# intellect4all/storage-engines

Measured on AMD Instinct MI355X. Metric: bloom build+probe Mkeys/s device-resident, 10M×16B keys @1% FPR, 1/2/4/8 GPU, higher is better.
Workload: dtype u64

## Files before the change

storage-engines_amd/csrc/seb_bucket.hip:

```cpp
#include <hip/hip_runtime.h>
#include <math.h>
#include <stdint.h>

#include "seb_device.h"
#include "seb_kernels.h"

namespace seb {

constexpr int kBktShift = 16;
constexpr uint32_t kBktWords = 1u << (kBktShift - 5);
constexpr uint32_t kMaxBuckets = 4096;
constexpr uint32_t kTilePos = 28672;
constexpr uint32_t kMaxTiles = 1024;
constexpr uint32_t kTargetTiles = 256;

__device__ __forceinline__ uint32_t block_exclusive_scan(uint32_t x, uint32_t *wsum, uint32_t *total) {
    const uint32_t lane = threadIdx.x & 63, wid = threadIdx.x >> 6, nw = blockDim.x >> 6;
    uint32_t v = x;
#pragma unroll
    for (int d = 1; d < 64; d <<= 1) {
        uint32_t y = __shfl_up(v, d, 64);
        if (lane >= (uint32_t)d) v += y;
    }
    if (lane == 63) wsum[wid] = v;
// ... 56 lines not shown
    for (uint64_t k0 = t0; k0 < t1; k0 += round_keys) {
        const uint64_t k1 = k0 + round_keys < t1 ? k0 + round_keys : t1;
        uint32_t pos[KP][KQ];
        bool valid[KP];
        if constexpr (KFIX > 0) {
#pragma unroll
            for (int r = 0; r < KP; ++r) {
                const uint64_t i = k0 + (uint64_t)r * blockDim.x + threadIdx.x;
                valid[r] = i < k1;
                if (valid[r]) {
                    if constexpr (IsPacked<Src>::value) {
                        static_assert(KFIX == 7, "packed residues are k == 7");
                        packed_positions((uint64_t)kv[r].x | (uint64_t)kv[r].y << 32, (uint32_t)md.m, (uint32_t)md.c,
                                         pos[r]);
                    } else {
                        uint64_t h1, h2;
                        if constexpr (kPre)
                            Src::hash_raw(kv[r], h1, h2);
                        else
                            src.hash(i, h1, h2);
                        for_positions<KFIX, true>(h1, h2, md, KFIX,
                                                  [&](uint32_t q, uint64_t p) { pos[r][q] = (uint32_t)p; });
                    }
#pragma unroll
                    for (int q = 0; q < KQ; ++q) atomicAdd(&cursor[pos[r][q] >> kBktShift], 1u);
                }
            }
            if (k1 < t1) prefetch(k1);
        } else {
            for (uint64_t i = k0 + threadIdx.x; i < k1; i += blockDim.x) {
                uint64_t h1, h2;
                src.hash(i, h1, h2);
                for_positions<0, true>(h1, h2, md, md.k,
                                       [&](uint32_t, uint64_t p) { atomicAdd(&cursor[(uint32_t)p >> kBktShift], 1u); });
            }
        }
        __syncthreads();
        {
            const uint32_t b0 = threadIdx.x * per;
            uint32_t c[8] = {0u, 0u, 0u, 0u, 0u, 0u, 0u, 0u}, s = 0;
            for (uint32_t j = 0; j < per; ++j)
                if (b0 + j < nb) {
                    c[j] = cursor[b0 + j];
                    s += c[j];
                }
            uint32_t tot;
            uint32_t pre = block_exclusive_scan(s, wsum, &tot);
            for (uint32_t j = 0; j < per; ++j)
                if (b0 + j < nb) {
                    cursor[b0 + j] = pre;
                    pre += c[j];
                }
        }
        __syncthreads();
        if constexpr (KFIX > 0) {
            uint32_t slot[KP][KQ];
#pragma unroll
            for (int r = 0; r < KP; ++r)
                if (valid[r]) {
#pragma unroll
                    for (int q = 0; q < KQ; ++q) slot[r][q] = atomicAdd(&cursor[pos[r][q] >> kBktShift], 1u);
                }
#pragma unroll
            for (int r = 0; r < KP; ++r)
                if (valid[r]) {
#pragma unroll
                    for (int q = 0; q < KQ; ++q) sorted[slot[r][q]] = pos[r][q];
                }
        } else {
            for (uint64_t i = k0 + threadIdx.x; i < k1; i += blockDim.x) {
                uint64_t h1, h2;
                src.hash(i, h1, h2);
                for_positions<0, true>(h1, h2, md, md.k, [&](uint32_t, uint64_t p) {
                    sorted[atomicAdd(&cursor[(uint32_t)p >> kBktShift], 1u)] = (uint32_t)p;
                });
            }
        }
        __syncthreads();
        for (uint32_t b = threadIdx.x; b < nb; b += blockDim.x) {
            const uint32_t start = b ? cursor[b - 1] : 0u, c = cursor[b] - start;
            const uint32_t reg = b * ntiles + t;
            if (fill[b] + c > cap) *ovf = 1u;
            fill[b] = reg * cap + fill[b] - start;
        }
        __syncthreads();
        const uint32_t cnt = (uint32_t)(k1 - k0) * md.k;
        if (*ovf == 0u) {
#pragma unroll 5
            for (uint32_t idx = threadIdx.x; idx < cnt; idx += blockDim.x) {
                const uint32_t p = sorted[idx];
                regions[fill[p >> kBktShift] + idx] = (uint16_t)p;
            }
        } else {
            for (uint32_t idx = threadIdx.x; idx < cnt; idx += blockDim.x) {
                const uint32_t p = sorted[idx];
                const uint32_t b = p >> kBktShift;
                const uint32_t e = fill[b] + idx;
                if (e - (b * ntiles + t) * cap < cap)
                    regions[e] = (uint16_t)p;
                else
                    __hip_atomic_fetch_or(ovw + (p >> 5), 1u << (p & 31), __ATOMIC_RELAXED, __HIP_MEMORY_SCOPE_AGENT);
            }
        }
        __syncthreads();
        for (uint32_t b = threadIdx.x; b < nb; b += blockDim.x) {
            fill[b] += cursor[b] - (b * ntiles + t) * cap;
            cursor[b] = 0u;
        }
        if (threadIdx.x == 0) *ovf = 0u;
        __syncthreads();
    }
    for (uint32_t b = threadIdx.x; b < nb; b += blockDim.x) counts[(uint64_t)b * ntiles + t] = fill[b];
}

constexpr uint32_t kBinMinBuckets = 512;
constexpr uint32_t kBinBig = 48, kBinSmall = 32;
constexpr uint32_t bin_lds_bytes(uint32_t nb, uint32_t slots) { return nb * (slots * 2 + 8) + 16; }
constexpr uint32_t kBinBigMaxBuckets = (160u * 1024 - 16) / (kBinBig * 2 + 8);
constexpr uint32_t kBinMaxBuckets = (160u * 1024 - 16) / (kBinSmall * 2 + 8);
constexpr double kBinMeanPos[2] = {20.0, 25.0};

__device__ __forceinline__ void bins_overflow_or(uint32_t *ovw, uint32_t b, uint32_t l) {
    const uint32_t p = (b << kBktShift) | l;
    __hip_atomic_fetch_or(ovw + (p >> 5), 1u << (p & 31), __ATOMIC_RELAXED, __HIP_MEMORY_SCOPE_AGENT);
}

template <typename Src, int THREADS, int KPT, uint32_t SB, int G = 1>
__global__ __launch_bounds__(THREADS) void k_bkt_scatter_bins(Src src, uint64_t n, ModArg md, uint32_t nb,
                                                              uint32_t tile_keys, uint32_t round_keys, uint32_t ntiles,
                                                              uint32_t cap, uint16_t *__restrict__ regions,
                                                              uint32_t *__restrict__ counts, uint32_t *__restrict__ ovw) {
    extern __shared__ uint4 smem4[];
    constexpr uint32_t S = SB, PAD = 8;
    static_assert(S % 8 == 0 && S <= 64, "a bucket's chunks must sit in one wave");
    uint16_t *bins = (uint16_t *)smem4;
    uint32_t *cnt = (uint32_t *)(bins + (size_t)nb * S);
    uint32_t *fill = cnt + nb;
    const uint32_t t = blockIdx.x;
    for (uint32_t b = threadIdx.x; b < nb; b += THREADS) {
        cnt[b] = 0u;
        fill[b] = 0u;
    }
    __syncthreads();
    const uint64_t t0 = (uint64_t)t * tile_keys;
    const uint64_t t1 = t0 + tile_keys < n ? t0 + tile_keys : n;
    constexpr bool kPre = SplitLoad<Src>::value;
    uint4 kv[kPre ? KPT : 1];
    auto prefetch = [&](uint64_t r0) {
        if constexpr (kPre) {
            const uint64_t r1 = r0 + round_keys < t1 ? r0 + round_keys : t1;
#pragma unroll
            for (int r = 0; r < KPT; ++r) {
                const uint64_t i = r0 + (uint64_t)r * THREADS + threadIdx.x;
                if (i < r1) kv[r] = src.load(i);
            }
        }
    };
    prefetch(t0);
    for (uint64_t k0 = t0; k0 < t1; k0 += round_keys) {
        const uint64_t k1 = k0 + round_keys < t1 ? k0 + round_keys : t1;
        constexpr int NSTEP = (KPT + G - 1) / G;
        uint32_t pp[G][7], ps[G][7];
        bool pv[G];
#pragma unroll
        for (int g = 0; g < G; ++g) pv[g] = false;
        auto write_bins = [&](const uint32_t (&pw)[7], const uint32_t (&sw)[7]) {
#pragma unroll
            for (int q = 0; q < 7; ++q) {
                const uint32_t p = pw[q], sl = sw[q], b = p >> kBktShift;
                bins[sl < S ? b * S + sl : nb * S + 4 * nb] = (uint16_t)p;
                if (sl >= S) {
                    const uint32_t e = fill[b] + sl;
                    if (e < cap)
                        regions[(uint64_t)(b * ntiles + t) * cap + e] = (uint16_t)p;
                    else
                        bins_overflow_or(ovw, b, p & 0xffffu);
                }
            }
        };
#pragma unroll
        for (int st = 0; st < NSTEP; ++st) {
            uint32_t pos[G][7], sl[G][7];
            bool valid[G];
#pragma unroll
            for (int g = 0; g < G; ++g) {
                const int r = st * G + g;
                const uint64_t i = k0 + (uint64_t)r * THREADS + threadIdx.x;
                valid[g] = r < KPT && i < k1;
                if (r < KPT && (kPre || valid[g])) {
                    if constexpr (IsPacked<Src>::value) {
                        packed_positions((uint64_t)kv[r].x | (uint64_t)kv[r].y << 32, (uint32_t)md.m, (uint32_t)md.c,
                                         pos[g]);
                    } else {
                        uint64_t h1, h2;
                        if constexpr (kPre)
                            Src::hash_raw(kv[r], h1, h2);
                        else
                            src.hash(i, h1, h2);
                        for_positions<7, true>(h1, h2, md, 7, [&](uint32_t q, uint64_t p) { pos[g][q] = (uint32_t)p; });
                    }
                }
            }
#pragma unroll
            for (int g = 0; g < G; ++g) {
                const int r = st * G + g;
                if (r >= KPT) continue;
                const uint64_t i = k0 + (uint64_t)r * THREADS + threadIdx.x;
                if constexpr (kPre) {
                    const uint64_t in = i + round_keys;
                    if (valid[g] && k1 < t1 && in < (k1 + round_keys < t1 ? k1 + round_keys : t1)) kv[r] = src.load(in);
                }
                if (valid[g]) {
#pragma unroll
                    for (int q = 0; q < 7; ++q) sl[g][q] = atomicAdd(&cnt[pos[g][q] >> kBktShift], 1u);
                }
            }
#pragma unroll
            for (int g = 0; g < G; ++g) {
                if (pv[g]) write_bins(pp[g], ps[g]);
#pragma unroll
                for (int q = 0; q < 7; ++q) {
                    pp[g][q] = pos[g][q];
                    ps[g][q] = sl[g][q];
                }
                pv[g] = valid[g];
            }
        }
#pragma unroll
        for (int g = 0; g < G; ++g)
            if (pv[g]) write_bins(pp[g], ps[g]);
        __syncthreads();
        {
            constexpr uint32_t NCH = S / 8, BPW = 64 / NCH, NW = THREADS / 64;
            const uint32_t lane = threadIdx.x & 63u, g = lane / NCH, j = lane - g * NCH;
            for (uint32_t b0 = (threadIdx.x >> 6) * BPW; b0 < nb; b0 += NW * BPW) {
                const uint32_t b = b0 + g;
                if (g >= BPW || b >= nb) continue;
                const uint32_t c = cnt[b], f = fill[b];
                const uint32_t rb = (b * ntiles + t) * cap;
                if (j * 8 < c) {
                    const uint4 w = *(const uint4 *)(bins + b * S + j * 8);
                    const uint32_t live = c - j * 8;
                    uint32_t ww[4] = {w.x, w.y, w.z, w.w};
                    const uint32_t e0 = w.x & 0xffffu, hi0 = e0 << 16;
#pragma unroll
                    for (uint32_t i = 0; i < 4; ++i)
                        ww[i] = 2 * i + 1 < live ? ww[i] : 2 * i < live ? (ww[i] & 0xffffu) | hi0 : e0 | hi0;
                    const uint32_t e = f + j * 8;
                    if (e < cap) {
                        *(uint4 *)(regions + rb + e) = make_uint4(ww[0], ww[1], ww[2], ww[3]);
                    } else {
#pragma unroll
                        for (uint32_t i = 0; i < 8; ++i) bins_overflow_or(ovw, b, (ww[i >> 1] >> ((i & 1) * 16)) & 0xffffu);
                    }
                }
                if (j == 0) {
                    const uint32_t padded = (c + (PAD - 1)) & ~(PAD - 1);
                    if (c > S) {
                        const uint16_t d = bins[b * S];
                        for (uint32_t e = f + c; e < f + padded; ++e)
                            if (e < cap) regions[(uint64_t)rb + e] = d;
                    }
                    cnt[b] = 0u;
                    fill[b] = f + padded;
                }
            }
        }
        __syncthreads();
    }
    for (uint32_t b = threadIdx.x; b < nb; b += THREADS) counts[(uint64_t)b * ntiles + t] = fill[b];
}

template <int THREADS, bool FRESH, bool PADDED = false>
__global__ __launch_bounds__(THREADS) void k_bkt_apply(const uint16_t *__restrict__ regions,
                                                   const uint32_t *__restrict__ counts, uint32_t ntiles, uint32_t cap,
                                                   uint32_t *__restrict__ words, uint64_t nwords,
                                                   uint32_t *__restrict__ ovf) {
    __shared__ uint32_t img[kBktWords];
    __shared__ uint32_t cnt[kMaxTiles];
    __shared__ uint32_t spilled, longest;
    const uint32_t b = blockIdx.x;
    for (uint32_t j = threadIdx.x; j < kBktWords; j += blockDim.x) img[j] = 0u;
    if (threadIdx.x == 0) {
        spilled = 0u;
        longest = 0u;
    }
    __syncthreads();
    for (uint32_t t = threadIdx.x; t < ntiles; t += blockDim.x) {
        const uint32_t c = counts[(uint64_t)b * ntiles + t];
        if (c > cap) spilled = 1u;
        cnt[t] = min(c, cap);
        atomicMax(&longest, min(c, cap));
    }
    __syncthreads();
    const uint32_t stride = cap / 8;
    const uint32_t chunks = (longest + 7) / 8;
    const uint32_t pairs = ntiles * chunks;
    const uint4 *reg = (const uint4 *)(regions + (uint64_t)b * ntiles * cap);
    constexpr uint32_t U = 4;
    for (uint32_t q0 = threadIdx.x; q0 < pairs; q0 += U * THREADS) {
        uint4 v[U];
#pragma unroll
        for (uint32_t u = 0; u < U; ++u) {
            const uint32_t q = q0 + u * THREADS;
            if (q < pairs) {
                const uint32_t t = q / chunks, c = q - t * chunks;
                v[u] = reg[t * stride + c];
            }
        }
#pragma unroll
        for (uint32_t u = 0; u < U; ++u) {
            const uint32_t q = q0 + u * THREADS;
            if (q >= pairs) break;
            const uint32_t t = q / chunks, c = q - t * chunks;
            const uint32_t valid = cnt[t];
            if (c * 8 < valid) {
                const uint32_t w[4] = {v[u].x, v[u].y, v[u].z, v[u].w};
#pragma unroll
                for (uint32_t e = 0; e < 8; ++e)
                    if (PADDED || c * 8 + e < valid) {
                        const uint32_t l = (w[e >> 1] >> ((e & 1) * 16)) & 0xffffu;
                        atomicOr(&img[l >> 5], 1u << (l & 31));
                    }
            }
        }
    }
    __syncthreads();
    const uint64_t w0 = (uint64_t)b * kBktWords;
    if constexpr (FRESH) {
        const bool sp = spilled != 0u;
        for (uint32_t j = threadIdx.x; j < kBktWords; j += blockDim.x)
            if (w0 + j < nwords) {
                uint32_t v = img[j];
                if (sp) {
                    v |= ovf[w0 + j];
                    ovf[w0 + j] = 0u;
                }
                words[w0 + j] = v;
            }
    } else {
        for (uint32_t j = threadIdx.x; j < kBktWords; j += blockDim.x) {
            const uint32_t v = img[j];
            if (v && w0 + j < nwords) words[w0 + j] |= v;
        }
    }
}


struct BktPlan {
    uint32_t nb, tile_keys, ntiles, cap;
    uint32_t round_keys;
    uint32_t bins;
    uint64_t off_regions, off_counts, bytes;
};

static uint32_t bin_slots(uint64_t m, uint32_t k) {
    const uint64_t nb = ((m + 31) / 32 + kBktWords - 1) / kBktWords;
    if (k != 7 || nb < kBinMinBuckets || nb > kBinMaxBuckets) return 0;
    return nb <= kBinBigMaxBuckets ? kBinBig : kBinSmall;
}
static uint32_t use_bins(uint64_t m, uint32_t k) { return options().scatter_bins ? bin_slots(m, k) : 0; }

constexpr uint32_t kScatterThreads = 1024;
static uint32_t scatter_kpt(uint32_t nb) {
    return ((uint64_t)kScatterThreads * 5 * 7 + 2 * nb + 17) * 4 <= 160u * 1024 ? 5u : 4u;
}

static BktPlan plan_bucketed(uint64_t n, uint64_t m, uint32_t k, uint32_t bins) {
    BktPlan p{};
    const uint64_t nwords = (m + 31) / 32;
    p.nb = (uint32_t)((nwords + kBktWords - 1) / kBktWords);
    p.bins = bins;
    const uint32_t thr = kScatterThreads;
    const uint32_t kpt = bins ? 5u : scatter_kpt(p.nb);
    const uint32_t pos = thr * kpt * 7;
    uint32_t round_keys = k == 7 ? kpt * thr : pos / k;
    if (bins) {
        const double mean = kBinMeanPos[bins == kBinBig];
        const uint64_t most = (uint64_t)(mean * (double)m / (double)(1u << kBktShift) / k);
        if (most < round_keys) round_keys = (uint32_t)(most > 64 ? most : 64);
    }
    const uint32_t target = kTargetTiles;
    uint64_t rounds_total = (n + round_keys - 1) / round_keys;
// ... 117 lines not shown
```

storage-engines_amd/csrc/seb_device.h:

```cpp
#pragma once
#include <hip/hip_runtime.h>
#include <stdint.h>

#include <type_traits>

#include "seb_kernels.h"

namespace seb {

constexpr uint64_t kFnvOffset = 0xcbf29ce484222325ull;
constexpr uint64_t kFnvPrime = 0x100000001b3ull;


__device__ __forceinline__ void fnv_byte(uint32_t b, uint64_t &h1, uint64_t &h2) {
    h1 = (h1 ^ (uint64_t)b) * kFnvPrime;
    h2 = (h2 * kFnvPrime) ^ (uint64_t)b;
}

__device__ __forceinline__ void fnv_word(uint32_t w, uint64_t &h1, uint64_t &h2) {
    fnv_byte(w & 0xffu, h1, h2);
    fnv_byte((w >> 8) & 0xffu, h1, h2);
    fnv_byte((w >> 16) & 0xffu, h1, h2);
    fnv_byte(w >> 24, h1, h2);
}
// ... 40 lines not shown
            break;
        default:
            asm("v_xor_b32_sdwa %0, %1, %2 dst_sel:DWORD dst_unused:UNUSED_PAD src0_sel:BYTE_3 src1_sel:DWORD"
                : "=v"(r) : "v"(w), "v"(a));
            break;
    }
    return r;
}

__device__ __forceinline__ void fnv_key16(const uint4 v, uint64_t &h1, uint64_t &h2) {
    const uint32_t w[4] = {v.x, v.y, v.z, v.w};
    uint32_t lo1 = (uint32_t)kFnvOffset, lo2 = (uint32_t)kFnvOffset;
    uint64_t acc1 = (uint32_t)(kFnvOffset >> 32) * pow435(16), acc2 = acc1;
#pragma unroll
    for (int j = 0; j < 16; ++j) {
        const uint32_t x = xor_byte(lo1, w[j >> 2], j & 3);
        const uint64_t p = (uint64_t)x * 435u;
        lo1 = (uint32_t)p;
        acc1 = mad_lo((uint32_t)(p >> 32) + (x << 8), pow435(15 - j), acc1);
        const uint64_t q = (uint64_t)lo2 * 435u;
        acc2 = mad_lo((uint32_t)(q >> 32) + (lo2 << 8), pow435(15 - j), acc2);
        lo2 = xor_byte((uint32_t)q, w[j >> 2], j & 3);
    }
    h1 = (acc1 << 32) | lo1;
    h2 = (acc2 << 32) | lo2;
}

struct FnvSplit {
    uint32_t lo1 = (uint32_t)kFnvOffset, lo2 = (uint32_t)kFnvOffset;
    uint64_t a1 = kFnvOffset >> 32, a2 = kFnvOffset >> 32;
    __device__ __forceinline__ void word(uint32_t w) {
        uint32_t d1[4], d2[4];
#pragma unroll
        for (int j = 0; j < 4; ++j) {
            const uint32_t x = xor_byte(lo1, w, j);
            const uint64_t p = (uint64_t)x * 435u;
            lo1 = (uint32_t)p;
            d1[j] = (uint32_t)(p >> 32) + (x << 8);
            const uint64_t q = (uint64_t)lo2 * 435u;
            d2[j] = (uint32_t)(q >> 32) + (lo2 << 8);
            lo2 = xor_byte((uint32_t)q, w, j);
        }
        const uint64_t t1 = mad_lo(d1[0], pow435(3), mad_lo(d1[1], pow435(2), mad_lo(d1[2], 435u, d1[3])));
        const uint64_t t2 = mad_lo(d2[0], pow435(3), mad_lo(d2[1], pow435(2), mad_lo(d2[2], 435u, d2[3])));
        a1 = mad_lo((uint32_t)a1, pow435(4), t1);
        a2 = mad_lo((uint32_t)a2, pow435(4), t2);
    }
    __device__ __forceinline__ void get(uint64_t &h1, uint64_t &h2) const {
        h1 = (a1 << 32) | lo1;
        h2 = (a2 << 32) | lo2;
    }
};

struct Keys16 {
    static constexpr bool kSplit = true;
    const uint4 *p;
    __device__ __forceinline__ uint64_t index(uint64_t i) const { return i; }
    __device__ __forceinline__ uint4 load(uint64_t i) const {
        typedef unsigned int u32x4 __attribute__((ext_vector_type(4)));
        const u32x4 v = __builtin_nontemporal_load((const u32x4 *)(p + i));
        return make_uint4(v.x, v.y, v.z, v.w);
    }
    __device__ __forceinline__ static void hash_raw(const uint4 v, uint64_t &h1, uint64_t &h2) { fnv_key16(v, h1, h2); }
    __device__ __forceinline__ void hash(uint64_t i, uint64_t &h1, uint64_t &h2) const { fnv_key16(load(i), h1, h2); }
};

struct KeysStrideW {
    const uint32_t *p;
    uint32_t words;
    __device__ __forceinline__ uint64_t index(uint64_t i) const { return i; }
    __device__ __forceinline__ void hash(uint64_t i, uint64_t &h1, uint64_t &h2) const {
        const uint32_t *k = p + i * words;
        h1 = kFnvOffset;
        h2 = kFnvOffset;
        for (uint32_t j = 0; j < words; ++j) fnv_word(k[j], h1, h2);
    }
};

struct KeysStrideB {
    const uint8_t *p;
    uint32_t stride;
    __device__ __forceinline__ uint64_t index(uint64_t i) const { return i; }
    __device__ __forceinline__ void hash(uint64_t i, uint64_t &h1, uint64_t &h2) const {
        const uint8_t *k = p + i * stride;
        h1 = kFnvOffset;
        h2 = kFnvOffset;
        for (uint32_t j = 0; j < stride; ++j) fnv_byte(k[j], h1, h2);
    }
};

__device__ __forceinline__ void fnv_range(const uint8_t *p, uint64_t s, uint64_t e, uint64_t &h1, uint64_t &h2) {
    h1 = kFnvOffset;
    h2 = kFnvOffset;
    uintptr_t a = ((uintptr_t)(p + s)) & ~(uintptr_t)3;
    const uintptr_t end = (uintptr_t)(p + e);
    const uintptr_t beg = (uintptr_t)(p + s);
    for (; a < end; a += 4) {
        const uint32_t w = *(const uint32_t *)a;
        const uint32_t lo = beg > a ? (uint32_t)(beg - a) : 0u;
        const uint32_t hi = end - a < 4 ? (uint32_t)(end - a) : 4u;
        if (lo == 0 && hi == 4)
            fnv_word(w, h1, h2);
        else
            fnv_word_part(w, lo, hi, h1, h2);
    }
}

struct KeysVar {
    const uint8_t *p;
    const uint64_t *off;
    __device__ __forceinline__ uint64_t index(uint64_t i) const { return i; }
    __device__ __forceinline__ void hash(uint64_t i, uint64_t &h1, uint64_t &h2) const {
        fnv_range(p, off[i], off[i + 1], h1, h2);
    }
};

struct KeysHashed {
    static constexpr bool kSplit = true;
    const uint4 *h;
    __device__ __forceinline__ uint64_t index(uint64_t i) const { return i; }
    __device__ __forceinline__ uint4 load(uint64_t i) const { return h[i]; }
    __device__ __forceinline__ static void hash_raw(const uint4 v, uint64_t &h1, uint64_t &h2) {
        h1 = (uint64_t)v.x | ((uint64_t)v.y << 32);
        h2 = (uint64_t)v.z | ((uint64_t)v.w << 32);
    }
    __device__ __forceinline__ void hash(uint64_t i, uint64_t &h1, uint64_t &h2) const { hash_raw(h[i], h1, h2); }
};

template <typename S, typename = void>
struct SplitLoad { static constexpr bool value = false; };
template <typename S>
struct SplitLoad<S, std::void_t<decltype(S::kSplit)>> { static constexpr bool value = S::kSplit; };


__device__ __forceinline__ uint64_t mod64(uint64_t x, uint64_t m, uint64_t mu) {
    uint64_t q = __umul64hi(x, mu);
    uint64_t r = x - q * m;
    r = r >= m ? r - m : r;
    r = r >= m ? r - m : r;
    return r;
}

__device__ __forceinline__ uint32_t mod_m31(uint64_t x, uint32_t m, uint64_t mu) {
    const uint32_t xl = (uint32_t)x, xh = (uint32_t)(x >> 32);
    const uint32_t ul = (uint32_t)mu, uh = (uint32_t)(mu >> 32);
    const uint64_t a = (uint64_t)xh * ul + __umulhi(xl, ul);
    const uint64_t b = (uint64_t)xl * uh + (uint32_t)a;
    const uint32_t qlo = xh * uh + (uint32_t)(a >> 32) + (uint32_t)(b >> 32);
    const uint32_t r = xl - qlo * m;
    const uint32_t s = r - m;
    return s < r ? s : r;
}

template <int KFIX, bool M32, typename F>
__device__ __forceinline__ void for_positions(uint64_t h1, uint64_t h2, const ModArg &md, uint32_t krt, F &&f) {
    const uint32_t k = KFIX > 0 ? (uint32_t)KFIX : krt;
    if (k == 0) return;
    uint64_t x = h1;
    if constexpr (M32) {
        const uint32_t m = (uint32_t)md.m, c = (uint32_t)md.c;
        uint32_t r = mod_m31(h1, m, md.mu);
        const uint32_t b = mod_m31(h2, m, md.mu);
        const uint32_t nb = m - b;
        const uint32_t bc = b >= c ? b - c : b + (m - c);
        const uint32_t nd = m - bc;
        f(0u, (uint64_t)r);
#pragma unroll
        for (uint32_t i = 1; i < k; ++i) {
            uint64_t xn = x + h2;
            const bool carry = xn < x;
            x = xn;
            const uint32_t na = carry ? nd : nb;
            const uint32_t t = r - na;
            r = r >= na ? t : t + m;
            f(i, (uint64_t)r);
        }
    } else {
        const uint64_t m = md.m, c = md.c;
        uint64_t r = mod64(h1, md.m, md.mu);
        const uint64_t b = mod64(h2, md.m, md.mu);
        f(0u, r);
#pragma unroll
        for (uint32_t i = 1; i < k; ++i) {
            uint64_t xn = x + h2;
            bool carry = xn < x;
            x = xn;
            uint64_t s = r + b;
            s = (s < r || s >= m) ? s - m : s;
            uint64_t t = s >= c ? s - c : s + (m - c);
            r = carry ? t : s;
            f(i, r);
        }
    }
}

template <typename Fn>
static inline hipError_t with_src(const KeyBatch &kb, Fn &&fn) {
    if (kb.hashes) return fn(KeysHashed{kb.hashes});
    if (kb.offsets) return fn(KeysVar{kb.data, kb.offsets});
    if (kb.stride == 16 && ((uintptr_t)kb.data & 15) == 0) return fn(Keys16{(const uint4 *)kb.data});
    if (kb.stride % 4 == 0 && ((uintptr_t)kb.data & 3) == 0)
        return fn(KeysStrideW{(const uint32_t *)kb.data, kb.stride / 4});
    return fn(KeysStrideB{kb.data, kb.stride});
}

__device__ __forceinline__ uint64_t pack_residue(uint64_t h1, uint64_t h2, const ModArg &md) {
    const uint64_t r0 = mod_m31(h1, (uint32_t)md.m, md.mu), b = mod_m31(h2, (uint32_t)md.m, md.mu);
    uint64_t f = 0, x = h1;
#pragma unroll
    for (uint32_t q = 1; q < 7; ++q) {
        const uint64_t xn = x + h2;
        f |= (uint64_t)(xn < x) << (q - 1);
        x = xn;
    }
    return r0 | (b << kPackBits) | (f << (2 * kPackBits));
}

__device__ __forceinline__ void packed_positions(uint64_t v, uint32_t m, uint32_t c, uint32_t pos[7]) {
    constexpr uint64_t kMask = (1ull << kPackBits) - 1;
    uint32_t x = (uint32_t)(v & kMask);
    const uint32_t b = (uint32_t)((v >> kPackBits) & kMask), f = (uint32_t)(v >> (2 * kPackBits));
    const uint32_t nb = m - b, bc = b >= c ? b - c : b + (m - c), nd = m - bc;
    pos[0] = x;
#pragma unroll
    for (int q = 1; q < 7; ++q) {
        const uint32_t na = (f >> (q - 1)) & 1u ? nd : nb;
        const uint32_t t = x - na;
        x = x >= na ? t : t + m;
        pos[q] = x;
    }
}

__device__ __forceinline__ uint64_t pack_residue6(uint64_t h1, uint64_t h2, const ModArg &md) {
    const uint64_t r0 = mod_m31(h1, (uint32_t)md.m, md.mu), b = mod_m31(h2, (uint32_t)md.m, md.mu);
    uint64_t f = 0, x = h1;
#pragma unroll
    for (uint32_t q = 1; q < 7; ++q) {
        const uint64_t xn = x + h2;
        f |= (uint64_t)(xn < x) << (q - 1);
        x = xn;
    }
    return r0 | (b << kPack6Bits) | (f << (2 * kPack6Bits));
}
__device__ __forceinline__ void store_packed6(uint8_t *base, uint64_t i, uint64_t v) {
    const uint64_t blk = i >> 6;
    const uint32_t lane = (uint32_t)i & 63u;
    __builtin_nontemporal_store((uint32_t)v, (uint32_t *)(base + blk * kPack6Block) + lane);
    __builtin_nontemporal_store((uint16_t)(v >> 32), (uint16_t *)(base + blk * kPack6Block + 256) + lane);
}
__device__ __forceinline__ uint64_t load_packed6(const uint8_t *base, uint64_t i) {
    const uint64_t blk = i >> 6;
    const uint32_t lane = (uint32_t)i & 63u;
    const uint32_t lo = __builtin_nontemporal_load((const uint32_t *)(base + blk * kPack6Block) + lane);
    const uint16_t hi = __builtin_nontemporal_load((const uint16_t *)(base + blk * kPack6Block + 256) + lane);
    return (uint64_t)lo | ((uint64_t)hi << 32);
}

struct KeysPacked {
    static constexpr bool kSplit = true;
    static constexpr bool kPacked = true;
    const uint64_t *p;
    __device__ __forceinline__ uint64_t index(uint64_t i) const { return i; }
    __device__ __forceinline__ uint4 load(uint64_t i) const {
        const uint64_t v = __builtin_nontemporal_load(p + i);
        return make_uint4((uint32_t)v, (uint32_t)(v >> 32), 0u, 0u);
    }
};

template <typename S, typename = void>
struct IsPacked { static constexpr bool value = false; };
template <typename S>
struct IsPacked<S, std::void_t<decltype(S::kPacked)>> { static constexpr bool value = S::kPacked; };

__device__ __forceinline__ uint64_t wave_peers(bool live, uint32_t v, uint32_t bits) {
    uint64_t peers = __ballot(live);
    for (uint32_t b = 0; b < bits; ++b) {
        const uint64_t on = __ballot(live && ((v >> b) & 1u));
        peers &= ((v >> b) & 1u) ? on : ~on;
    }
    return peers;
}

__device__ __forceinline__ uint32_t lanes_below(uint64_t mask) {
    return __builtin_amdgcn_mbcnt_hi((uint32_t)(mask >> 32), __builtin_amdgcn_mbcnt_lo((uint32_t)mask, 0u));
}

}
```

storage-engines_amd/csrc/seb_kernels.hip:

```cpp
#include <hip/hip_runtime.h>
#include <stdint.h>

#include <algorithm>

#include <type_traits>

#include "seb_device.h"
#include "seb_kernels.h"

namespace seb {


template <typename Src, int KFIX, bool M32>
__global__ __launch_bounds__(256) void k_build(Src src, uint64_t n, uint32_t *__restrict__ words, ModArg md) {
    const uint64_t stride = (uint64_t)gridDim.x * blockDim.x;
    for (uint64_t i = (uint64_t)blockIdx.x * blockDim.x + threadIdx.x; i < n; i += stride) {
        uint64_t h1, h2;
        src.hash(i, h1, h2);
        for_positions<KFIX, M32>(h1, h2, md, md.k, [&](uint32_t, uint64_t p) {
            __hip_atomic_fetch_or(words + (p >> 5), 1u << (uint32_t)(p & 31), __ATOMIC_RELAXED,
                                  __HIP_MEMORY_SCOPE_AGENT);
        });
    }
}
// ... 2 lines not shown
__global__ __launch_bounds__(256) void k_probe(Src src, uint64_t n, const uint32_t *__restrict__ words, ModArg md,
                                               uint8_t *__restrict__ out) {
    if constexpr (KFIX > 0) {
        using P = typename std::conditional<M32, uint32_t, uint64_t>::type;
        constexpr int S = (SPLIT > 0 && SPLIT < KFIX) ? SPLIT : KFIX;
        const uint64_t span = (uint64_t)blockDim.x * KPT;
        for (uint64_t base = (uint64_t)blockIdx.x * span; base < n; base += (uint64_t)gridDim.x * span) {
            P pos[KPT][KFIX];
            uint32_t acc[KPT];
#pragma unroll
            for (int r = 0; r < KPT; ++r) {
                const uint64_t i = base + (uint64_t)r * blockDim.x + threadIdx.x;
                uint64_t h1 = 0, h2 = 0;
                if (i < n) src.hash(i, h1, h2);
                for_positions<KFIX, M32>(h1, h2, md, KFIX, [&](uint32_t q, uint64_t p) { pos[r][q] = (P)p; });
                acc[r] = i < n ? 1u : 0u;
            }
#pragma unroll
            for (int r = 0; r < KPT; ++r)
#pragma unroll
                for (int q = 0; q < S; ++q)
                    if (acc[r]) acc[r] &= words[pos[r][q] >> 5] >> (uint32_t)(pos[r][q] & 31);
            if constexpr (S < KFIX) {
#pragma unroll
                for (int r = 0; r < KPT; ++r)
                    if (acc[r] & 1u) {
#pragma unroll
                        for (int q = S; q < KFIX; ++q) acc[r] &= words[pos[r][q] >> 5] >> (uint32_t)(pos[r][q] & 31);
                    }
            }
#pragma unroll
            for (int r = 0; r < KPT; ++r) {
                const uint64_t i = base + (uint64_t)r * blockDim.x + threadIdx.x;
                if (i < n) out[src.index(i)] = (uint8_t)(acc[r] & 1u);
            }
        }
    } else {
        const uint64_t stride = (uint64_t)gridDim.x * blockDim.x;
        for (uint64_t i = (uint64_t)blockIdx.x * blockDim.x + threadIdx.x; i < n; i += stride) {
            uint64_t h1, h2;
            src.hash(i, h1, h2);
            uint32_t acc = 1u;
            for_positions<0, M32>(h1, h2, md, md.k, [&](uint32_t, uint64_t p) {
                if (acc & 1u) acc &= words[p >> 5] >> (uint32_t)(p & 31);
            });
            out[src.index(i)] = (uint8_t)(acc & 1u);
        }
    }
}

template <typename Src, int KPT>
__global__ __launch_bounds__(256) void k_probe_sliced(Src src, uint64_t n, const uint32_t *__restrict__ words,
                                                      ModArg md, uint8_t *__restrict__ out, uint32_t slice_shift,
                                                      uint32_t nslices) {
    const uint64_t span = (uint64_t)blockDim.x * KPT;
    for (uint64_t base = (uint64_t)blockIdx.x * span; base < n; base += (uint64_t)gridDim.x * span) {
        uint32_t pos[KPT][7];
        uint32_t acc[KPT];
#pragma unroll
        for (int r = 0; r < KPT; ++r) {
            const uint64_t i = base + (uint64_t)r * blockDim.x + threadIdx.x;
            uint64_t h1 = 0, h2 = 0;
            if (i < n) src.hash(i, h1, h2);
            for_positions<7, true>(h1, h2, md, 7, [&](uint32_t q, uint64_t p) { pos[r][q] = (uint32_t)p; });
            acc[r] = i < n ? 1u : 0u;
        }
        for (uint32_t sl = 0; sl < nslices; ++sl) {
#pragma unroll
            for (int r = 0; r < KPT; ++r)
#pragma unroll
                for (int q = 0; q < 7; ++q) {
                    const uint32_t w = pos[r][q] >> 5;
                    if ((acc[r] & 1u) && (w >> slice_shift) == sl) acc[r] &= words[w] >> (pos[r][q] & 31);
                }
        }
#pragma unroll
        for (int r = 0; r < KPT; ++r) {
            const uint64_t i = base + (uint64_t)r * blockDim.x + threadIdx.x;
            if (i < n) out[src.index(i)] = (uint8_t)(acc[r] & 1u);
        }
    }
}

template <typename Src>
__global__ __launch_bounds__(256) void k_pack_residues(Src src, uint64_t n, ModArg md, uint64_t *__restrict__ out) {
    const uint64_t stride = (uint64_t)gridDim.x * blockDim.x;
    for (uint64_t i = (uint64_t)blockIdx.x * blockDim.x + threadIdx.x; i < n; i += stride) {
        uint64_t h1, h2;
        src.hash(i, h1, h2);
        out[src.index(i)] = pack_residue(h1, h2, md);
    }
}

template <typename Src>
__global__ __launch_bounds__(256) void k_pack_residues6(Src src, uint64_t n, ModArg md, uint8_t *__restrict__ out) {
    const uint64_t stride = (uint64_t)gridDim.x * blockDim.x;
    for (uint64_t i = (uint64_t)blockIdx.x * blockDim.x + threadIdx.x; i < n; i += stride) {
        uint64_t h1, h2;
        src.hash(i, h1, h2);
        store_packed6(out, i, pack_residue6(h1, h2, md));
    }
}

template <typename Src, int KPT>
__global__ __launch_bounds__(256) void k_probe_sliced_emit(Src src, uint64_t n, const uint32_t *__restrict__ words,
                                                           ModArg md, uint8_t *__restrict__ out,
                                                           uint64_t *__restrict__ packed, uint32_t slice_shift,
                                                           uint32_t nslices) {
    const uint64_t span = (uint64_t)blockDim.x * KPT;
    for (uint64_t base = (uint64_t)blockIdx.x * span; base < n; base += (uint64_t)gridDim.x * span) {
        uint32_t pos[KPT][7];
        uint32_t acc[KPT];
#pragma unroll
        for (int r = 0; r < KPT; ++r) {
            const uint64_t i = base + (uint64_t)r * blockDim.x + threadIdx.x;
            uint64_t h1 = 0, h2 = 0;
            if (i < n) src.hash(i, h1, h2);
            const uint64_t pw = pack_residue(h1, h2, md);
            packed_positions(pw, (uint32_t)md.m, (uint32_t)md.c, pos[r]);
            acc[r] = i < n ? 1u : 0u;
            if (i < n) __builtin_nontemporal_store(pw, packed + src.index(i));
        }
        for (uint32_t sl = 0; sl < nslices; ++sl) {
#pragma unroll
            for (int r = 0; r < KPT; ++r)
#pragma unroll
                for (int q = 0; q < 7; ++q) {
                    const uint32_t w = pos[r][q] >> 5;
                    if ((acc[r] & 1u) && (w >> slice_shift) == sl) acc[r] &= words[w] >> (pos[r][q] & 31);
                }
        }
#pragma unroll
        for (int r = 0; r < KPT; ++r) {
            const uint64_t i = base + (uint64_t)r * blockDim.x + threadIdx.x;
            if (i < n) out[src.index(i)] = (uint8_t)(acc[r] & 1u);
        }
    }
}

constexpr unsigned kPhaseBlock = 256;
template <typename Src, int KPT>
__global__ __launch_bounds__(kPhaseBlock) void k_probe_phase0(Src src, uint64_t n, const uint32_t *__restrict__ words,
                                                      ModArg md, uint8_t *__restrict__ out,
                                                      uint64_t *__restrict__ packed, uint32_t hi) {
    const uint64_t span = (uint64_t)blockDim.x * KPT;
    for (uint64_t base = (uint64_t)blockIdx.x * span; base < n; base += (uint64_t)gridDim.x * span) {
        uint32_t pos[KPT][7];
        uint32_t acc[KPT];
#pragma unroll
        for (int r = 0; r < KPT; ++r) {
            const uint64_t i = base + (uint64_t)r * blockDim.x + threadIdx.x;
            uint64_t h1 = 0, h2 = 0;
            if (i < n) src.hash(i, h1, h2);
            const uint64_t pw = pack_residue(h1, h2, md);
            packed_positions(pw, (uint32_t)md.m, (uint32_t)md.c, pos[r]);
            acc[r] = i < n ? 1u : 0u;
            if (i < n) __builtin_nontemporal_store(pw, packed + i);
        }
#pragma unroll
        for (int r = 0; r < KPT; ++r)
#pragma unroll
            for (int q = 0; q < 7; ++q) {
                const uint32_t w = pos[r][q] >> 5;
                if ((acc[r] & 1u) && w < hi) acc[r] &= words[w] >> (pos[r][q] & 31);
            }
#pragma unroll
        for (int r = 0; r < KPT; ++r) {
            const uint64_t i = base + (uint64_t)r * blockDim.x + threadIdx.x;
            if (i < n) out[i] = (uint8_t)(acc[r] & 1u);
        }
    }
}

__global__ __launch_bounds__(kPhaseBlock) void k_probe_phase(const uint64_t *__restrict__ packed, uint64_t n,
                                                     const uint32_t *__restrict__ words, ModArg md,
                                                     uint8_t *__restrict__ out, uint32_t lo, uint32_t hi,
                                                     uint32_t first) {
    const uint32_t m = (uint32_t)md.m, c = (uint32_t)md.c;
    constexpr uint64_t kMask = (1ull << kPackBits) - 1;
    const uint64_t stride = (uint64_t)gridDim.x * blockDim.x * 4;
    for (uint64_t i0 = ((uint64_t)blockIdx.x * blockDim.x + threadIdx.x) * 4; i0 < n; i0 += stride) {
        const bool full = i0 + 4 <= n;
        uint32_t a;
        if (first) {
            a = full ? 0x01010101u : 0x01010101u & ((1u << (8 * (uint32_t)(n - i0))) - 1u);
        } else if (full) {
            a = *(const uint32_t *)(out + i0);
        } else {
            a = 0;
            for (uint32_t r = 0; i0 + r < n; ++r) a |= (uint32_t)out[i0 + r] << (8 * r);
        }
        if (a == 0u) continue;
        uint64_t pv[4];
        if (full) {
            typedef unsigned int u32x4 __attribute__((ext_vector_type(4)));
            const u32x4 p0 = __builtin_nontemporal_load((const u32x4 *)(packed + i0));
            const u32x4 p1 = __builtin_nontemporal_load((const u32x4 *)(packed + i0 + 2));
            pv[0] = (uint64_t)p0.x | ((uint64_t)p0.y << 32);
            pv[1] = (uint64_t)p0.z | ((uint64_t)p0.w << 32);
            pv[2] = (uint64_t)p1.x | ((uint64_t)p1.y << 32);
            pv[3] = (uint64_t)p1.z | ((uint64_t)p1.w << 32);
        } else {
#pragma unroll
            for (uint32_t r = 0; r < 4; ++r) pv[r] = i0 + r < n ? packed[i0 + r] : 0ull;
        }
        uint32_t na = a;
#pragma unroll
        for (uint32_t r = 0; r < 4; ++r) {
            uint32_t live = (a >> (8 * r)) & 1u;
            uint32_t x = (uint32_t)(pv[r] & kMask);
            const uint32_t b = (uint32_t)((pv[r] >> kPackBits) & kMask), f = (uint32_t)(pv[r] >> (2 * kPackBits));
            const uint32_t nb = m - b, bc = b >= c ? b - c : b + (m - c), nd = m - bc;
#pragma unroll
            for (int q = 0; q < 7; ++q) {
                if (q > 0) {
                    const uint32_t d = (f >> (q - 1)) & 1u ? nd : nb;
                    const uint32_t t = x - d;
                    x = x >= d ? t : t + m;
                }
                const uint32_t w = x >> 5;
                if (live && w >= lo && w < hi) live &= words[w] >> (x & 31);
            }
            na &= ~((((a >> (8 * r)) & 1u) & (live ^ 1u)) << (8 * r));
        }
        if (na != a || first) {
            if (full)
                *(uint32_t *)(out + i0) = na;
            else
                for (uint32_t r = 0; i0 + r < n; ++r) out[i0 + r] = (uint8_t)(na >> (8 * r));
        }
    }
}

template <typename Src>
__global__ __launch_bounds__(kPhaseBlock) void k_probe_c0(Src src, uint64_t n, const uint32_t *__restrict__ words,
                                                  ModArg md, uint64_t *__restrict__ rows,
                                                  ulonglong2 *__restrict__ recs, uint32_t hi) {
    const uint32_t lane = threadIdx.x & 63u;
    for (uint64_t base = (uint64_t)blockIdx.x * blockDim.x; base < n; base += (uint64_t)gridDim.x * blockDim.x) {
        const uint64_t i = base + threadIdx.x;
        uint32_t pos[7];
        uint64_t pw;
        if constexpr (IsPacked<Src>::value) {
            const uint4 v = i < n ? src.load(i) : make_uint4(0u, 0u, 0u, 0u);
            pw = (uint64_t)v.x | (uint64_t)v.y << 32;
            packed_positions(pw, (uint32_t)md.m, (uint32_t)md.c, pos);
        } else {
            uint64_t h1 = 0, h2 = 0;
            if (i < n) src.hash(i, h1, h2);
            pw = pack_residue(h1, h2, md);
            packed_positions(pw, (uint32_t)md.m, (uint32_t)md.c, pos);
        }
        uint32_t acc = i < n ? 1u : 0u;
#pragma unroll
        for (int q = 0; q < 7; ++q) {
            const uint32_t w = pos[q] >> 5;
            if ((acc & 1u) && w < hi) acc &= words[w] >> (pos[q] & 31);
        }
        const uint64_t alive = __ballot(acc & 1u);
        const uint64_t g = i >> 6;
        if (acc & 1u) __builtin_nontemporal_store(pw, rows + g * 64 + lanes_below(alive));
        if (lane == 0 && i < n) recs[g] = make_ulonglong2(alive, alive);
    }
}

__device__ __forceinline__ uint64_t uniform64(uint64_t v) {
    const uint32_t lo = (uint32_t)__builtin_amdgcn_readfirstlane((uint32_t)v);
    const uint32_t hi = (uint32_t)__builtin_amdgcn_readfirstlane((uint32_t)(v >> 32));
    return (uint64_t)hi << 32 | lo;
}

template <int G, bool LAST>
__global__ __launch_bounds__(kPhaseBlock) void k_probe_cp(const uint64_t *__restrict__ rows, ulonglong2 *recs,
                                                  uint64_t n, const uint32_t *__restrict__ words, ModArg md,
                                                  uint8_t *__restrict__ out, uint32_t lo, uint32_t hi) {
    const uint32_t m = (uint32_t)md.m, c = (uint32_t)md.c;
    constexpr uint64_t kMask = (1ull << kPackBits) - 1;
    const uint32_t lane = threadIdx.x & 63u;
    const uint64_t below = (1ull << lane) - 1ull;
    const uint64_t ng = (n + 63) >> 6;
    const uint64_t wave = __builtin_amdgcn_readfirstlane((blockIdx.x * blockDim.x + threadIdx.x) >> 6);
    const uint64_t step = (uint64_t)gridDim.x * (blockDim.x >> 6) * G;
    for (uint64_t g0 = wave * G; g0 < ng; g0 += step) {
        uint64_t m0[G], lv[G], pv[G];
        uint32_t live[G];
        struct Recs { ulonglong2 r[G]; };
        const Recs rv = *(const Recs *)(recs + g0);
#pragma unroll
        for (int j = 0; j < G; ++j) {
            const bool in = g0 + j < ng;
            m0[j] = in ? uniform64(rv.r[j].x) : 0ull;
            lv[j] = in ? uniform64(rv.r[j].y) : 0ull;
            live[j] = (uint32_t)(lv[j] >> lane) & 1u;
        }
#pragma unroll
        for (int j = 0; j < G; ++j)
            pv[j] = live[j] ? __builtin_nontemporal_load(rows + (g0 + j) * 64 + __popcll(m0[j] & below)) : 0ull;
#pragma unroll
        for (int j = 0; j < G; ++j) {
            uint32_t x = (uint32_t)(pv[j] & kMask);
            const uint32_t b = (uint32_t)((pv[j] >> kPackBits) & kMask), f = (uint32_t)(pv[j] >> (2 * kPackBits));
            const uint32_t nb = m - b, bc = b >= c ? b - c : b + (m - c), nd = m - bc;
#pragma unroll
            for (int q = 0; q < 7; ++q) {
                if (q > 0) {
                    const uint32_t d = (f >> (q - 1)) & 1u ? nd : nb;
                    const uint32_t t = x - d;
                    x = x >= d ? t : t + m;
                }
                const uint32_t w = x >> 5;
                if (live[j] && w >= lo && w < hi) live[j] &= words[w] >> (x & 31);
            }
        }
#pragma unroll
        for (int j = 0; j < G; ++j) {
            const uint64_t g = g0 + j;
            if constexpr (LAST) {
                const uint64_t i = g * 64 + lane;
                if (g < ng && i < n) out[i] = (uint8_t)live[j];
            } else {
                const uint64_t nl = __ballot(live[j]);
                if (lane == 0 && g < ng && nl != lv[j]) recs[g].y = nl;
            }
        }
    }
}

template <int KPT>
__global__ __launch_bounds__(256) void k_probe_packed(const uint64_t *__restrict__ packed, uint64_t n,
                                                      const uint32_t *__restrict__ words, ModArg md,
                                                      uint8_t *__restrict__ out, uint32_t slice_shift,
                                                      uint32_t nslices) {
    const uint32_t m = (uint32_t)md.m, c = (uint32_t)md.c;
    constexpr uint64_t kMask = (1ull << kPackBits) - 1;
    const uint64_t span = (uint64_t)blockDim.x * KPT;
    for (uint64_t base = (uint64_t)blockIdx.x * span; base < n; base += (uint64_t)gridDim.x * span) {
        uint32_t pos[KPT][7];
        uint32_t acc[KPT];
#pragma unroll
        for (int r = 0; r < KPT; ++r) {
            const uint64_t i = base + (uint64_t)r * blockDim.x + threadIdx.x;
            const uint64_t v = i < n ? __builtin_nontemporal_load(packed + i) : 0ull;
            uint32_t x = (uint32_t)(v & kMask);
            const uint32_t b = (uint32_t)((v >> kPackBits) & kMask), f = (uint32_t)(v >> (2 * kPackBits));
            const uint32_t nb = m - b, bc = b >= c ? b - c : b + (m - c), nd = m - bc;
            pos[r][0] = x;
#pragma unroll
            for (int q = 1; q < 7; ++q) {
                const uint32_t na = (f >> (q - 1)) & 1u ? nd : nb;
                const uint32_t t = x - na;
                x = x >= na ? t : t + m;
                pos[r][q] = x;
            }
            acc[r] = i < n ? 1u : 0u;
        }
        for (uint32_t sl = 0; sl < nslices; ++sl) {
#pragma unroll
            for (int r = 0; r < KPT; ++r)
#pragma unroll
                for (int q = 0; q < 7; ++q) {
                    const uint32_t w = pos[r][q] >> 5;
                    if ((acc[r] & 1u) && (w >> slice_shift) == sl) acc[r] &= words[w] >> (pos[r][q] & 31);
                }
        }
#pragma unroll
        for (int r = 0; r < KPT; ++r) {
            const uint64_t i = base + (uint64_t)r * blockDim.x + threadIdx.x;
            if (i < n) out[i] = (uint8_t)(acc[r] & 1u);
        }
    }
}

template <typename Src, typename MaskT, bool SAME, int KFIX, bool M32>
__global__ __launch_bounds__(256) void k_probe_multi(Src src, uint64_t n, MultiArg ma, MaskT *__restrict__ mask) {
    const uint64_t stride = (uint64_t)gridDim.x * blockDim.x;
    for (uint64_t i = (uint64_t)blockIdx.x * blockDim.x + threadIdx.x; i < n; i += stride) {
        uint64_t h1, h2;
        src.hash(i, h1, h2);
        MaskT w = 0;
        if constexpr (SAME) {
            uint64_t pos[KFIX > 0 ? KFIX : 1];
            if constexpr (KFIX > 0) {
                for_positions<KFIX, M32>(h1, h2, ma.f[0].md, KFIX, [&](uint32_t q, uint64_t p) { pos[q] = p; });
                for (uint32_t f = 0; f < ma.nf; ++f) {
                    const uint32_t *wd = ma.f[f].words;
                    uint32_t acc = 1u;
#pragma unroll
                    for (int q = 0; q < KFIX; ++q)
                        if (acc & 1u) acc &= wd[pos[q] >> 5] >> (uint32_t)(pos[q] & 31);
                    w |= (MaskT)(acc & 1u) << f;
                }
            }
        } else {
            for (uint32_t f = 0; f < ma.nf; ++f) {
                const uint32_t *wd = ma.f[f].words;
                uint32_t acc = 1u;
                for_positions<KFIX, M32>(h1, h2, ma.f[f].md, ma.f[f].md.k, [&](uint32_t, uint64_t p) {
                    if (acc & 1u) acc &= wd[p >> 5] >> (uint32_t)(p & 31);
                });
                w |= (MaskT)(acc & 1u) << f;
            }
        }
        mask[src.index(i)] = w;
    }
}

template <typename MaskT>
__global__ __launch_bounds__(256) void k_interleave(MultiArg ma, uint64_t m, MaskT *__restrict__ table) {
    const uint64_t p = (uint64_t)blockIdx.x * blockDim.x + threadIdx.x;
    if (p >= m) return;
    const uint64_t w = p >> 5;
    const uint32_t j = (uint32_t)(p & 31);
    MaskT e = 0;
    for (uint32_t f0 = 0; f0 < ma.nf; f0 += 16) {
        uint32_t v[16];
#pragma unroll
        for (uint32_t r = 0; r < 16; ++r) v[r] = f0 + r < ma.nf ? ma.f[f0 + r].words[w] : 0u;
#pragma unroll
        for (uint32_t r = 0; r < 16; ++r) e |= (MaskT)((v[r] >> j) & 1u) << ((f0 + r) & (8 * sizeof(MaskT) - 1));
    }
    table[p] = e;
}

__device__ __forceinline__ uint64_t wave_transpose64(uint64_t x, uint32_t lane) {
    constexpr uint64_t kLow[6] = {0x00000000FFFFFFFFull, 0x0000FFFF0000FFFFull, 0x00FF00FF00FF00FFull,
                                  0x0F0F0F0F0F0F0F0Full, 0x3333333333333333ull, 0x5555555555555555ull};
#pragma unroll
    for (int st = 0; st < 6; ++st) {
        const uint32_t j = 32u >> st;
        const uint64_t lo = kLow[st];
        const uint32_t ylo = (uint32_t)__shfl_xor((int)(uint32_t)x, (int)j, 64);
        const uint32_t yhi = (uint32_t)__shfl_xor((int)(uint32_t)(x >> 32), (int)j, 64);
        const uint64_t y = (uint64_t)yhi << 32 | ylo;
        x = (lane & j) ? (x & ~lo) | ((y & ~lo) >> j) : (x & lo) | ((y & lo) << j);
    }
    return x;
}

template <typename MaskT>
__global__ __launch_bounds__(256) void k_interleave_xpose(MultiArg ma, uint64_t m, MaskT *__restrict__ table) {
    const uint32_t lane = threadIdx.x & 63u;
    const uint64_t p0 = (((uint64_t)blockIdx.x * blockDim.x + threadIdx.x) >> 6) * 128;
    if (p0 >= m) return;
    uint4 v = make_uint4(0u, 0u, 0u, 0u);
    if (lane < ma.nf) v = *(const uint4 *)(ma.f[lane].words + (p0 >> 5));
#pragma unroll
    for (int h = 0; h < 2; ++h) {
        const uint64_t x = h ? (uint64_t)v.w << 32 | v.z : (uint64_t)v.y << 32 | v.x;
        const uint64_t e = wave_transpose64(x, lane);
        const uint64_t p = p0 + 64 * h + lane;
        if (p < m) table[p] = (MaskT)e;
    }
}

template <typename MaskT>
static void launch_interleave(const MultiArg &ma, uint64_t m, MaskT *table, hipStream_t s) {
    bool aligned = true;
    for (uint32_t f = 0; f < ma.nf; ++f) aligned &= ((uintptr_t)ma.f[f].words & 15) == 0;
    if (aligned)
        hipLaunchKernelGGL((k_interleave_xpose<MaskT>), dim3((unsigned)((m + 511) / 512)), dim3(256), 0, s, ma, m, table);
    else
        hipLaunchKernelGGL((k_interleave<MaskT>), dim3((unsigned)((m + 255) / 256)), dim3(256), 0, s, ma, m, table);
}

template <typename Src, typename MaskT, int KPT>
__global__ __launch_bounds__(256) void k_probe_interleaved(Src src, uint64_t n, const MaskT *__restrict__ table, ModArg md,
                                                           MaskT *__restrict__ mask, uint32_t slice_shift,
                                                           uint32_t nslices) {
    const uint64_t span = (uint64_t)blockDim.x * KPT;
    for (uint64_t base = (uint64_t)blockIdx.x * span; base < n; base += (uint64_t)gridDim.x * span) {
        uint32_t pos[KPT][7];
        MaskT acc[KPT];
#pragma unroll
        for (int r = 0; r < KPT; ++r) {
            const uint64_t i = base + (uint64_t)r * blockDim.x + threadIdx.x;
            uint64_t h1 = 0, h2 = 0;
            if (i < n) src.hash(i, h1, h2);
            for_positions<7, true>(h1, h2, md, 7, [&](uint32_t q, uint64_t p) { pos[r][q] = (uint32_t)p; });
            acc[r] = i < n ? (MaskT)~(MaskT)0 : (MaskT)0;
        }
        for (uint32_t sl = 0; sl < nslices; ++sl) {
#pragma unroll
            for (int r = 0; r < KPT; ++r)
#pragma unroll
                for (int q = 0; q < 7; ++q)
                    if (acc[r] && (pos[r][q] >> slice_shift) == sl) acc[r] &= table[pos[r][q]];
        }
#pragma unroll
        for (int r = 0; r < KPT; ++r) {
            const uint64_t i = base + (uint64_t)r * blockDim.x + threadIdx.x;
            if (i < n) mask[src.index(i)] = acc[r];
        }
    }
}

template <typename MaskT, int W>
__global__ __launch_bounds__(256) void k_probe_interleaved_packed(const void *__restrict__ packed, uint64_t n,
                                                                  const MaskT *__restrict__ table, ModArg md,
                                                                  MaskT *__restrict__ mask, uint32_t slice_shift,
                                                                  uint32_t nslices) {
    constexpr int KPT = 2;
    constexpr uint32_t kBits = W == 8 ? kPackBits : kPack6Bits;
    constexpr uint64_t kMask = (1ull << kBits) - 1;
    const uint32_t m = (uint32_t)md.m, c = (uint32_t)md.c;
// ... 582 lines not shown
```

Measured before the change: 45530.

## Use branchless min/bfi modular steps and fuse hashing with position packing

Replaces the compare-and-select modular subtraction in the double-hashing position generator with v_min_u32 / v_max_u32 / v_bfi_b32 inline assembly. Adds a hashed_positions helper that produces the seven positions and the packed residue word in a single pass, so the separate pack_residue and packed_positions calls are no longer both needed. In the bucket build kernel, the bin writes become unconditional with a dummy slot, and the rare spill path into per-tile regions becomes a non-unrolled loop that runs only when a slot overflows. The aim is to cut VALU instructions and divergent branches in the hot loops, at the cost of extra dummy stores and target-specific assembly.

```diff
diff --git a/storage-engines_amd/csrc/seb_bucket.hip b/storage-engines_amd/csrc/seb_bucket.hip
--- a/storage-engines_amd/csrc/seb_bucket.hip
+++ b/storage-engines_amd/csrc/seb_bucket.hip
@@ -232,7 +232,7 @@
 #pragma unroll
             for (int r = 0; r < KPT; ++r) {
                 const uint64_t i = r0 + (uint64_t)r * THREADS + threadIdx.x;
-                if (i < r1) kv[r] = src.load(i);
+                kv[r] = src.load(i < r1 ? i : r0);
             }
         }
     };
@@ -244,17 +244,26 @@
         bool pv[G];
 #pragma unroll
         for (int g = 0; g < G; ++g) pv[g] = false;
-        auto write_bins = [&](const uint32_t (&pw)[7], const uint32_t (&sw)[7]) {
+        auto write_bins = [&](bool on, const uint32_t (&pw)[7], const uint32_t (&sw)[7]) {
+            uint32_t most = 0u;
 #pragma unroll
             for (int q = 0; q < 7; ++q) {
                 const uint32_t p = pw[q], sl = sw[q], b = p >> kBktShift;
-                bins[sl < S ? b * S + sl : nb * S + 4 * nb] = (uint16_t)p;
-                if (sl >= S) {
-                    const uint32_t e = fill[b] + sl;
-                    if (e < cap)
-                        regions[(uint64_t)(b * ntiles + t) * cap + e] = (uint16_t)p;
-                    else
-                        bins_overflow_or(ovw, b, p & 0xffffu);
+                bins[on ? (sl < S ? b * S + sl : nb * S + 4 * nb) : nb * S + 4 * nb] = (uint16_t)p;
+                most = most > sl ? most : sl;
+            }
+            if (on && most >= S) {
+#pragma nounroll
+                for (int q = 0; q < 7; ++q) {
+                    uint32_t p = pw[0], sl = sw[0];
+#pragma unroll
+                    for (int j = 1; j < 7; ++j) {
+                        p = q == j ? pw[j] : p;
+                        sl = q == j ? sw[j] : sl;
+                    }
+                    const uint32_t b = p >> kBktShift, e = fill[b] + sl;
+                    if (sl >= S && e < cap) regions[(uint64_t)(b * ntiles + t) * cap + e] = (uint16_t)p;
+                    if (sl >= S && e >= cap) bins_overflow_or(ovw, b, p & 0xffffu);
                 }
             }
         };
@@ -290,6 +299,8 @@
                     const uint64_t in = i + round_keys;
                     if (valid[g] && k1 < t1 && in < (k1 + round_keys < t1 ? k1 + round_keys : t1)) kv[r] = src.load(in);
                 }
+#pragma unroll
+                for (int q = 0; q < 7; ++q) sl[g][q] = 0u;
                 if (valid[g]) {
 #pragma unroll
                     for (int q = 0; q < 7; ++q) sl[g][q] = atomicAdd(&cnt[pos[g][q] >> kBktShift], 1u);
@@ -297,7 +308,7 @@
             }
 #pragma unroll
             for (int g = 0; g < G; ++g) {
-                if (pv[g]) write_bins(pp[g], ps[g]);
+                if (st > 0) write_bins(pv[g], pp[g], ps[g]);
 #pragma unroll
                 for (int q = 0; q < 7; ++q) {
                     pp[g][q] = pos[g][q];
@@ -308,7 +319,7 @@
         }
 #pragma unroll
         for (int g = 0; g < G; ++g)
-            if (pv[g]) write_bins(pp[g], ps[g]);
+            write_bins(pv[g], pp[g], ps[g]);
         __syncthreads();
         {
             constexpr uint32_t NCH = S / 8, BPW = 64 / NCH, NW = THREADS / 64;
diff --git a/storage-engines_amd/csrc/seb_device.h b/storage-engines_amd/csrc/seb_device.h
--- a/storage-engines_amd/csrc/seb_device.h
+++ b/storage-engines_amd/csrc/seb_device.h
@@ -216,6 +216,28 @@
     return s < r ? s : r;
 }
 
+__device__ __forceinline__ uint32_t step_mod(uint32_t x, uint32_t na, uint32_t m) {
+    const uint32_t t = x - na, u = t + m;
+    uint32_t r;
+    asm("v_min_u32 %0, %1, %2" : "=v"(r) : "v"(t), "v"(u));
+    return r;
+}
+
+__device__ __forceinline__ void step_addends(uint32_t b, uint32_t m, uint32_t c, uint32_t &nb, uint32_t &nd) {
+    nb = m - b;
+    const uint32_t t = b - c, u = t - m;
+    uint32_t mnd;
+    asm("v_max_u32 %0, %1, %2" : "=v"(mnd) : "v"(t), "v"(u));
+    nd = 0u - mnd;
+}
+
+__device__ __forceinline__ uint32_t pick_addend(uint32_t f, int bit, uint32_t nb, uint32_t nd) {
+    const uint32_t mask = (uint32_t)((int32_t)(f << (31 - bit)) >> 31);
+    uint32_t r;
+    asm("v_bfi_b32 %0, %1, %2, %3" : "=v"(r) : "v"(mask), "v"(nd), "v"(nb));
+    return r;
+}
+
 template <int KFIX, bool M32, typename F>
 __device__ __forceinline__ void for_positions(uint64_t h1, uint64_t h2, const ModArg &md, uint32_t krt, F &&f) {
     const uint32_t k = KFIX > 0 ? (uint32_t)KFIX : krt;
@@ -225,18 +247,15 @@
         const uint32_t m = (uint32_t)md.m, c = (uint32_t)md.c;
         uint32_t r = mod_m31(h1, m, md.mu);
         const uint32_t b = mod_m31(h2, m, md.mu);
-        const uint32_t nb = m - b;
-        const uint32_t bc = b >= c ? b - c : b + (m - c);
-        const uint32_t nd = m - bc;
+        uint32_t nb, nd;
+        step_addends(b, m, c, nb, nd);
         f(0u, (uint64_t)r);
 #pragma unroll
         for (uint32_t i = 1; i < k; ++i) {
-            uint64_t xn = x + h2;
-            const bool carry = xn < x;
+            unsigned long long xn;
+            const bool carry = __builtin_uaddll_overflow(x, h2, &xn);
             x = xn;
-            const uint32_t na = carry ? nd : nb;
-            const uint32_t t = r - na;
-            r = r >= na ? t : t + m;
+            r = step_mod(r, carry ? nd : nb, m);
             f(i, (uint64_t)r);
         }
     } else {
@@ -284,15 +303,35 @@
     constexpr uint64_t kMask = (1ull << kPackBits) - 1;
     uint32_t x = (uint32_t)(v & kMask);
     const uint32_t b = (uint32_t)((v >> kPackBits) & kMask), f = (uint32_t)(v >> (2 * kPackBits));
-    const uint32_t nb = m - b, bc = b >= c ? b - c : b + (m - c), nd = m - bc;
+    uint32_t nb, nd;
+    step_addends(b, m, c, nb, nd);
     pos[0] = x;
 #pragma unroll
     for (int q = 1; q < 7; ++q) {
-        const uint32_t na = (f >> (q - 1)) & 1u ? nd : nb;
-        const uint32_t t = x - na;
-        x = x >= na ? t : t + m;
+        x = step_mod(x, pick_addend(f, q - 1, nb, nd), m);
         pos[q] = x;
     }
+}
+
+__device__ __forceinline__ uint64_t hashed_positions(uint64_t h1, uint64_t h2, const ModArg &md, uint32_t pos[7]) {
+    const uint32_t m = (uint32_t)md.m;
+    uint32_t x = mod_m31(h1, m, md.mu);
+    const uint32_t r0 = x, b = mod_m31(h2, m, md.mu);
+    uint32_t nb, nd;
+    step_addends(b, m, (uint32_t)md.c, nb, nd);
+    unsigned long long s = h1;
+    uint32_t f = 0;
+    pos[0] = x;
+#pragma unroll
+    for (int q = 1; q < 7; ++q) {
+        const bool carry = __builtin_uaddll_overflow(s, h2, &s);
+        f |= (uint32_t)carry << (q - 1);
+        x = step_mod(x, carry ? nd : nb, m);
+        pos[q] = x;
+    }
+    static_assert(2 * kPackBits == 58 && kPackBits < 32, "the flags sit in bits 26-31 of the high word");
+    const uint32_t lo = r0 | (b << kPackBits), hi = (b >> (32 - kPackBits)) | (f << (2 * kPackBits - 32));
+    return (uint64_t)hi << 32 | lo;
 }
 
 __device__ __forceinline__ uint64_t pack_residue6(uint64_t h1, uint64_t h2, const ModArg &md) {
diff --git a/storage-engines_amd/csrc/seb_kernels.hip b/storage-engines_amd/csrc/seb_kernels.hip
--- a/storage-engines_amd/csrc/seb_kernels.hip
+++ b/storage-engines_amd/csrc/seb_kernels.hip
@@ -178,8 +178,7 @@
             const uint64_t i = base + (uint64_t)r * blockDim.x + threadIdx.x;
             uint64_t h1 = 0, h2 = 0;
             if (i < n) src.hash(i, h1, h2);
-            const uint64_t pw = pack_residue(h1, h2, md);
-            packed_positions(pw, (uint32_t)md.m, (uint32_t)md.c, pos[r]);
+            const uint64_t pw = hashed_positions(h1, h2, md, pos[r]);
             acc[r] = i < n ? 1u : 0u;
             if (i < n) __builtin_nontemporal_store(pw, packed + i);
         }
@@ -236,14 +235,11 @@
             uint32_t live = (a >> (8 * r)) & 1u;
             uint32_t x = (uint32_t)(pv[r] & kMask);
             const uint32_t b = (uint32_t)((pv[r] >> kPackBits) & kMask), f = (uint32_t)(pv[r] >> (2 * kPackBits));
-            const uint32_t nb = m - b, bc = b >= c ? b - c : b + (m - c), nd = m - bc;
+            uint32_t nb, nd;
+            step_addends(b, m, c, nb, nd);
 #pragma unroll
             for (int q = 0; q < 7; ++q) {
-                if (q > 0) {
-                    const uint32_t d = (f >> (q - 1)) & 1u ? nd : nb;
-                    const uint32_t t = x - d;
-                    x = x >= d ? t : t + m;
-                }
+                if (q > 0) x = step_mod(x, pick_addend(f, q - 1, nb, nd), m);
                 const uint32_t w = x >> 5;
                 if (live && w >= lo && w < hi) live &= words[w] >> (x & 31);
             }
@@ -274,8 +270,7 @@
         } else {
             uint64_t h1 = 0, h2 = 0;
             if (i < n) src.hash(i, h1, h2);
-            pw = pack_residue(h1, h2, md);
-            packed_positions(pw, (uint32_t)md.m, (uint32_t)md.c, pos);
+            pw = hashed_positions(h1, h2, md, pos);
         }
         uint32_t acc = i < n ? 1u : 0u;
 #pragma unroll
@@ -326,14 +321,11 @@
         for (int j = 0; j < G; ++j) {
             uint32_t x = (uint32_t)(pv[j] & kMask);
             const uint32_t b = (uint32_t)((pv[j] >> kPackBits) & kMask), f = (uint32_t)(pv[j] >> (2 * kPackBits));
-            const uint32_t nb = m - b, bc = b >= c ? b - c : b + (m - c), nd = m - bc;
+            uint32_t nb, nd;
+            step_addends(b, m, c, nb, nd);
 #pragma unroll
             for (int q = 0; q < 7; ++q) {
-                if (q > 0) {
-                    const uint32_t d = (f >> (q - 1)) & 1u ? nd : nb;
-                    const uint32_t t = x - d;
-                    x = x >= d ? t : t + m;
-                }
+                if (q > 0) x = step_mod(x, pick_addend(f, q - 1, nb, nd), m);
                 const uint32_t w = x >> 5;
                 if (live[j] && w >= lo && w < hi) live[j] &= words[w] >> (x & 31);
             }
@@ -369,13 +361,12 @@
             const uint64_t v = i < n ? __builtin_nontemporal_load(packed + i) : 0ull;
             uint32_t x = (uint32_t)(v & kMask);
             const uint32_t b = (uint32_t)((v >> kPackBits) & kMask), f = (uint32_t)(v >> (2 * kPackBits));
-            const uint32_t nb = m - b, bc = b >= c ? b - c : b + (m - c), nd = m - bc;
+            uint32_t nb, nd;
+            step_addends(b, m, c, nb, nd);
             pos[r][0] = x;
 #pragma unroll
             for (int q = 1; q < 7; ++q) {
-                const uint32_t na = (f >> (q - 1)) & 1u ? nd : nb;
-                const uint32_t t = x - na;
-                x = x >= na ? t : t + m;
+                x = step_mod(x, pick_addend(f, q - 1, nb, nd), m);
                 pos[r][q] = x;
             }
             acc[r] = i < n ? 1u : 0u;
```

Result: faster. 46240 (median of 6 runs) (+1.5%).
